# Asherchi/Stereo_Match_Traditional

Hardware: AMD Instinct MI355X
Metric: Mdisparities/s (HxWxD/s) + ms/pair, AD-Census 1920x1080 D=192 (higher is better)
Workload: dtype f32; 1 GPU; AD-Census 9x7 both views + WTA, 1920x1080 D=192 (adcensus_1080p_d192); parallelism=pairs sharded over 1 GPU(s), backend=none (single process), ranks_joined=1, ranks_joined_how=all_reduce(SUM) of 1 per rank over the job's communicator, world_size=1, launcher=none

## Files before the change

stereo_match_traditional_amd/csrc/adcensus.hip:

```cpp
#include "smt_common.h"
#include "adcensus_internal.h"
#include <math.h>
#include <stdlib.h>
#include <string.h>
#include <algorithm>
#include <new>
#include <type_traits>

namespace {

constexpr int TJ = 64;
constexpr int NT = 256;

struct Tables {
    uint64_t *cenA[2];
    uint64_t *cenX[2];
    uint64_t *mask;
    uint8_t *u8[2];
    float *lut;
    uint16_t *rank;
    int *flag;
    int WX;
    int edge_col;
    unsigned long long *stamp;
// ... 1257 lines not shown
        const vecf<C> x = *reinterpret_cast<const vecf<C> *>(c);
#pragma unroll
        for (int k = 0; k < C; k++) v[k] = x.v[k];
    } else {
#pragma unroll
        for (int k = 0; k < C; k++) v[k] = (dl + k < D) ? c[k] : INFINITY;
    }
    const int wd = wave_wta<C, FULL>(v, dl, D);
    if (lane == 0) disp[p] = (float)wd;
}

}

thread_local int g_smt_last_hip = 0;

struct smt_adcensus {
    int device;
    int H, W, D;
    float sigmaC, sigmaS;
    hipStream_t stream;
    float *vol[2];
    Tables T;
    Tables TS[2];
    hipStream_t prep_stream;
    hipEvent_t in_ready, prep_done[2], cost_done[2];
    long n_pairs;
    hipEvent_t *ev;
    bool timing;
    bool force_generic;
    long n_timed;
    long n_seen;
    int timing_stride;
    bool *ev_merged;
    bool plain_stores;
    float store_mode_ms[2];
    int place_tries;
    float place_ms;
    unsigned long long *skeys[2];
    bool conv_pending;
    int conv_map;
    float *conv_dR;
    bool vol_lent, vol_pending;
    int maps_resident[3];
};

SMT_API const char *smt_strerror(int s)
{
    switch (s) {
    case SMT_OK: return "ok";
    case SMT_ERR_ARG: return "invalid argument";
    case SMT_ERR_HIP: return "HIP runtime error";
    case SMT_ERR_ALLOC: return "device allocation failed";
    case SMT_ERR_DOMAIN: return "image values outside the integer 0..255 domain";
    case SMT_ERR_REF_UB: return "reference behaviour undefined for these inputs";
    case SMT_ERR_STATE: return "call order violated";
    default: return "unknown status";
// ... 180 lines not shown
            kv[a * 64 + c] = ((uint64_t)bits << 32) | (uint32_t)(a * 64 + c);
        }
    std::sort(kv, kv + RANK_N);
    int r = -1;
    uint32_t prev = 0;
    for (int n = 0; n < RANK_N; n++) {
        const uint32_t bits = (uint32_t)(kv[n] >> 32);
        if (n == 0 || bits != prev) r++;
        prev = bits;
        rank[(uint32_t)kv[n]] = (uint16_t)r;
    }
    delete[] kv;
    return true;
}

static void flush_conversion(smt_adcensus *h)
{
    if (!h->conv_pending) return;
    const long N = (long)h->H * h->W;
    hipLaunchKernelGGL(k_shared_convert, dim3((unsigned)shared_conv_items(h->H, h->W)), dim3(NT), 0, h->stream,
                       h->skeys[h->conv_map], h->conv_dR, N);
    h->conv_pending = false;
}

template <int C, bool FULL>
static void query_maps_resident(smt_adcensus *h, int cus)
{
    int n[3] = {0, 0, 0};
    if (hipOccupancyMaxActiveBlocksPerMultiprocessor(&n[0], k_cost_maps_shared<C, FULL>, NT, 0) != hipSuccess) n[0] = 0;
    if (hipOccupancyMaxActiveBlocksPerMultiprocessor(&n[1], k_cost_maps2p<C, FULL, MODE_MAPS_FLOAT>, NT, 0) != hipSuccess) n[1] = 0;
    if (hipOccupancyMaxActiveBlocksPerMultiprocessor(&n[2], k_cost_maps2p<C, FULL, MODE_MAPS_RANK>, NT, 0) != hipSuccess) n[2] = 0;
    for (int t = 0; t < 3; t++) h->maps_resident[t] = n[t] > 0 ? cus / 8 * n[t] : 0;
}
static void set_maps_resident(smt_adcensus *h)
{
    h->maps_resident[0] = h->maps_resident[1] = h->maps_resident[2] = 0;
    int cus = 0;
// ... 10 lines not shown
    default: break;
    }
    (void)hipGetLastError();
}

static int adcensus_create(int H, int W, int D, float sigmaC, float sigmaS, unsigned flags, smt_adcensus **out)
{
    if (!out || H <= 0 || W <= 0 || D <= 0 || D > SMT_MAX_DISPARITY || !(sigmaC > 0.0f) || !(sigmaS > 0.0f) ||
        (long long)H * W >= (1ll << 31))
        return SMT_ERR_ARG;
    smt_adcensus *h = new (std::nothrow) smt_adcensus();
    if (!h) return SMT_ERR_ALLOC;
    h->device = smt_current_device();
    h->H = H; h->W = W; h->D = D; h->sigmaC = sigmaC; h->sigmaS = sigmaS;
    h->stream = nullptr; h->timing = false; h->force_generic = false; h->ev = nullptr; h->n_timed = 0; h->n_seen = 0; h->timing_stride = 1; h->ev_merged = nullptr;
    h->n_pairs = 0;
    const size_t N = (size_t)H * W, V = N * D;
    const int WX = W + 4;
    int rc = place_volumes(h, !(flags & SMT_ADCENSUS_NO_PLACEMENT_SEARCH));
    auto alloc = [&](void **p, size_t bytes) { if (rc == SMT_OK) rc = smt_malloc(p, bytes); };
    alloc((void **)&h->TS[0].lut, 320 * 4);
    alloc((void **)&h->TS[0].rank, RANK_N * 2);
    alloc((void **)&h->TS[0].flag, 4);
    for (int t = 0; t < 2; t++) {
        h->TS[t].WX = WX;
        h->TS[t].stamp = nullptr;
        h->TS[t].lut = h->TS[0].lut;
        h->TS[t].rank = h->TS[0].rank;
        h->TS[t].flag = h->TS[0].flag;
        for (int v = 0; v < 2; v++) {
            alloc((void **)&h->TS[t].cenA[v], N * 8);
            alloc((void **)&h->TS[t].cenX[v], (size_t)H * WX * 8);
            alloc((void **)&h->TS[t].u8[v], N);
        }
        alloc((void **)&h->TS[t].mask, N * 8);
    }
    for (int t = 0; t < 2; t++) alloc((void **)&h->skeys[t], N * 8);
    h->T = h->TS[0];
    if (rc != SMT_OK) { smt_adcensus_destroy(h); return rc; }
    if (hipStreamCreateWithFlags(&h->prep_stream, hipStreamNonBlocking) != hipSuccess ||
        hipEventCreateWithFlags(&h->in_ready, hipEventDisableTiming) != hipSuccess) {
        smt_adcensus_destroy(h);
        return SMT_ERR_HIP;
    }
    for (int t = 0; t < 2; t++)
        if (hipEventCreateWithFlags(&h->prep_done[t], hipEventDisableTiming) != hipSuccess ||
            hipEventCreateWithFlags(&h->cost_done[t], hipEventDisableTiming) != hipSuccess) {
            smt_adcensus_destroy(h);
            return SMT_ERR_HIP;
        }
    float lut[320];
    build_lut(sigmaC, sigmaS, lut);
    uint16_t *rank = new (std::nothrow) uint16_t[RANK_N];
    if (!rank || !build_rank(lut, rank)) { delete[] rank; smt_adcensus_destroy(h); return SMT_ERR_ALLOC; }
    const bool rank_ok = hipMemcpy(h->TS[0].rank, rank, RANK_N * 2, hipMemcpyHostToDevice) == hipSuccess;
    delete[] rank;
    if (!rank_ok || hipMemcpy(h->TS[0].lut, lut, sizeof(lut), hipMemcpyHostToDevice) != hipSuccess ||
        hipMemset(h->vol[0], 0, V * 4) != hipSuccess || hipMemset(h->vol[1], 0, V * 4) != hipSuccess ||
        hipMemset(h->TS[0].flag, 0, 4) != hipSuccess || hipMemset(h->skeys[0], 0xFF, N * 8) != hipSuccess ||
        hipMemset(h->skeys[1], 0xFF, N * 8) != hipSuccess) {
        smt_adcensus_destroy(h);
        return SMT_ERR_HIP;
    }
    calibrate_store_mode(h, !(flags & SMT_ADCENSUS_NO_STORE_CALIBRATION));
    set_maps_resident(h);
    *out = h;
    return SMT_OK;
}

SMT_API int smt_adcensus_create(int H, int W, int D, float sigmaC, float sigmaS, smt_adcensus **out)
{
    return adcensus_create(H, W, D, sigmaC, sigmaS, 0u, out);
}

SMT_API int smt_adcensus_create_ex(int device, int H, int W, int D, float sigmaC, float sigmaS, unsigned flags, smt_adcensus **out)
{
    if (flags & ~(unsigned)(SMT_ADCENSUS_NO_PLACEMENT_SEARCH | SMT_ADCENSUS_NO_STORE_CALIBRATION)) return SMT_ERR_ARG;
    if (device < 0) return adcensus_create(H, W, D, sigmaC, sigmaS, flags, out);
// ... 3 lines not shown
    return adcensus_create(H, W, D, sigmaC, sigmaS, flags, out);
}

SMT_API int smt_adcensus_create_on(int device, int H, int W, int D, float sigmaC, float sigmaS, smt_adcensus **out)
{
    int n = 0;
    if (hipGetDeviceCount(&n) != hipSuccess || device < 0 || device >= n) return SMT_ERR_ARG;
    smt_dev_guard dev_guard(device);
    return smt_adcensus_create(H, W, D, sigmaC, sigmaS, out);
}

SMT_API int smt_adcensus_destroy(smt_adcensus *h)
{
    if (!h) return SMT_ERR_ARG;
    smt_dev_guard dev_guard(h->device);
    if (h->conv_pending) { flush_conversion(h); (void)hipStreamSynchronize(h->stream); }
    if (h->prep_stream) { (void)hipStreamSynchronize(h->prep_stream); (void)hipStreamDestroy(h->prep_stream); }
    if (h->in_ready) (void)hipEventDestroy(h->in_ready);
    for (int t = 0; t < 2; t++) {
        if (h->prep_done[t]) (void)hipEventDestroy(h->prep_done[t]);
        if (h->cost_done[t]) (void)hipEventDestroy(h->cost_done[t]);
    }
    (void)hipFree(h->vol[0]); (void)hipFree(h->vol[1]);
    for (int t = 0; t < 2; t++) {
        for (int v = 0; v < 2; v++) {
            (void)hipFree(h->TS[t].cenA[v]); (void)hipFree(h->TS[t].cenX[v]); (void)hipFree(h->TS[t].u8[v]);
        }
        (void)hipFree(h->TS[t].mask);
    }
    (void)hipFree(h->TS[0].lut); (void)hipFree(h->TS[0].rank); (void)hipFree(h->TS[0].flag);
    (void)hipFree(h->skeys[0]); (void)hipFree(h->skeys[1]);
    if (h->ev) {
        for (int k = 0; k < SMT_TIMING_SLOTS * 4; k++) (void)hipEventDestroy(h->ev[k]);
        delete[] h->ev_merged;
        delete[] h->ev;
    }
    delete h;
    return SMT_OK;
}

SMT_API int smt_adcensus_set_stream(smt_adcensus *h, void *s)
{
    if (!h) return SMT_ERR_ARG;
    smt_dev_guard dev_guard(h->device);
    h->stream = smt_stream(s);
    return SMT_OK;
}

SMT_API int smt_adcensus_set_quirks(smt_adcensus *h, unsigned quirks)
{
    if (!h || (quirks & ~SMT_QUIRK_FIX_ALL)) return SMT_ERR_ARG;
    const int col = (quirks & SMT_QUIRK_FIX_CENSUS_RIGHT_EDGE) ? h->W - 1 : 0;
    h->T.edge_col = h->TS[0].edge_col = h->TS[1].edge_col = col;
    return SMT_OK;
}

template <int C, bool FULL>
static void launch_cost(smt_adcensus *h, int view0, int nviews, float *d0, float *d1)
{
    const int D = h->D;
    dim3 grid((h->W + TJ - 1) / TJ, h->H, nviews);
    const int NX = TJ + D;
    size_t shm = (size_t)NX * 8 + TJ * 16 + 320 * 4 + NX + TJ;
    shm = (shm + 15) & ~(size_t)15;
    hipLaunchKernelGGL((k_cost<C, FULL>), grid, dim3(NT), shm, h->stream, h->H, h->W, D, h->T,
                       view0, h->vol[0], h->vol[1], d0, d1);
}

static int maps_chunks()
{
    const char *env = getenv("SMT_MAPS_CHUNKS");
    const int k = env ? atoi(env) : 0;
    return k >= 1 && k <= 64 ? k : 4;
}

constexpr int TAPER_N2_HALVES = 0, TAPER_N1_HALVES = 2;
static void maps_taper(int S, long per, int K, int &n2, int &n1)
{
    n2 = n1 = 0;
    const char *env = getenv("SMT_MAPS_TAPER");
// ... 32 lines not shown
    return !(env && env[0] == 'r') && dL && dR && maps_shared_shape(h->W, h->D) && maps_shared();
}

static int prep_items(int H, int W, int &ptx)
{
    ptx = (W + PTW - 1) / PTW;
    const int pty = (H + PTH - 1) / PTH, eb = (H + PNT / 16 - 1) / (PNT / 16);
    return ptx * (pty + (eb + ptx - 1) / ptx);
}

template <int C, bool FULL>
static void launch_fast(smt_adcensus *h, int views, float *dL, float *dR, const float *nL, const float *nR, bool maps)
{
    const int nbx = (h->W + FTJ - 1) / FTJ;
    auto blocks = [&](int nviews) { return dim3((unsigned)(((long)nbx * h->H * nviews + 7) / 8 * 8)); };
    if (views == SMT_VIEW_BOTH && maps) {
        const int K = maps_chunks();
        int nprep = 0, ptx = 1;
        if (nL) nprep = prep_items(h->H, h->W, ptx);
        const Tables &Tn = h->TS[(h->n_pairs + 1) & 1];
        const char *env = getenv("SMT_MAPS_KERNEL");
        int n2, n1;
        if (pair_takes_shared(h, views, dL, dR, maps)) {
            const int km = (int)(h->n_pairs & 1);
            if (h->conv_pending && h->conv_map == km) flush_conversion(h);
            const bool carried = h->conv_pending;
            maps_taper(h->maps_resident[0], ((long)nbx * h->H + 7) >> 3, K, n2, n1);
            const int ncs = maps_groups(nbx, h->H, 1, K, n2, n1), Dd = FULL ? 64 * C : h->D;
            const int cbody = maps_body_groups(nbx, h->H, 1, K, n2, n1);
            const int nconv = carried ? shared_conv_items(h->H, h->W) : 0, nedge = shared_edge_items(h->H, h->W, Dd);
            const unsigned gs = 8u * (unsigned)fused_grid(ncs, nprep + nconv + nedge, cbody).groups;
            hipLaunchKernelGGL((k_cost_maps_shared<C, FULL>), dim3(gs), dim3(NT), 0, h->stream, h->H, h->W, h->D, h->T, dL, dR,
                               h->skeys[km], nbx, K, shared_pub_hi(h->W), ncs, nprep, nL, nR, Tn, ptx, nconv, nedge,
                               carried ? h->skeys[h->conv_map] : nullptr, carried ? h->conv_dR : nullptr, n2, n1, cbody);
            if (SMT_SHARED_KNOCKOUT != 2) { h->conv_pending = true; h->conv_map = km; h->conv_dR = dR; }
            else h->conv_pending = false;
            if (shared_finish_apart()) flush_conversion(h);
            return;
        }
        const bool rank = env && env[0] == 'r';
        maps_taper(h->maps_resident[rank ? 2 : 1], ((long)nbx * h->H * 2 + 7) >> 3, K, n2, n1);
        const int ncost = maps_groups(nbx, h->H, 2, K, n2, n1), cbody = maps_body_groups(nbx, h->H, 2, K, n2, n1);
        const unsigned grid = nL ? 8u * (unsigned)fused_grid(ncost, nprep, cbody).groups : (unsigned)ncost;
        if (rank)
            hipLaunchKernelGGL((k_cost_maps2p<C, FULL, MODE_MAPS_RANK>), dim3(grid), dim3(NT), 0, h->stream, h->H, h->W,
                               h->D, h->T, dL, dR, nbx, K, ncost, nprep, nL, nR, Tn, ptx, n2, n1, cbody);
        else
            hipLaunchKernelGGL((k_cost_maps2p<C, FULL, MODE_MAPS_FLOAT>), dim3(grid), dim3(NT), 0, h->stream, h->H, h->W,
                               h->D, h->T, dL, dR, nbx, K, ncost, nprep, nL, nR, Tn, ptx, n2, n1, cbody);
        return;
    }
    if (views == SMT_VIEW_BOTH && nL) {
        const int ncost = (int)blocks(2).x;
        const int ptx = (h->W + PTW - 1) / PTW, pty = (h->H + PTH - 1) / PTH;
        const int eb = (h->H + PNT / 16 - 1) / (PNT / 16);
        const int nprep = ptx * (pty + (eb + ptx - 1) / ptx);
        const unsigned grid = 8u * (unsigned)fused_grid(ncost, nprep).groups;
        const Tables &Tn = h->TS[(h->n_pairs + 1) & 1];
        if (h->plain_stores)
            hipLaunchKernelGGL((k_cost_fast2p<C, FULL, false>), dim3(grid), dim3(NT), 0, h->stream, h->H, h->W, h->D, h->T,
                               h->vol[0], h->vol[1], dL, dR, nbx, ncost, nprep, nL, nR, Tn, ptx);
        else
            hipLaunchKernelGGL((k_cost_fast2p<C, FULL, true>), dim3(grid), dim3(NT), 0, h->stream, h->H, h->W, h->D, h->T,
                               h->vol[0], h->vol[1], dL, dR, nbx, ncost, nprep, nL, nR, Tn, ptx);
        return;
    }
    if (views == SMT_VIEW_BOTH) {
        if (h->plain_stores)
            hipLaunchKernelGGL((k_cost_fast2<C, FULL, false>), blocks(2), dim3(NT), 0, h->stream, h->H, h->W, h->D, h->T, h->vol[0],
                               h->vol[1], dL, dR, nbx);
        else
            hipLaunchKernelGGL((k_cost_fast2<C, FULL, true>), blocks(2), dim3(NT), 0, h->stream, h->H, h->W, h->D, h->T, h->vol[0],
                               h->vol[1], dL, dR, nbx);
        return;
    }
    if (views & SMT_VIEW_LEFT)
        hipLaunchKernelGGL((k_cost_fast<C, 0, FULL>), blocks(1), dim3(NT), 0, h->stream, h->H, h->W, h->D, h->T,
                           h->vol[0], dL, nbx);
    if (views & SMT_VIEW_RIGHT)
        hipLaunchKernelGGL((k_cost_fast<C, 1, FULL>), blocks(1), dim3(NT), 0, h->stream, h->H, h->W, h->D, h->T,
                           h->vol[1], dR, nbx);
}

static bool launch_fast_as(int C, bool full, smt_adcensus *h, int views, float *dL, float *dR, const float *nL,
                           const float *nR, bool maps)
{
    switch (C * 2 + (full ? 1 : 0)) {
    case 3: launch_fast<1, true>(h, views, dL, dR, nL, nR, maps); break;
    case 5: launch_fast<2, true>(h, views, dL, dR, nL, nR, maps); break;
    case 7: launch_fast<3, true>(h, views, dL, dR, nL, nR, maps); break;
    case 9: launch_fast<4, true>(h, views, dL, dR, nL, nR, maps); break;
    case 2: launch_fast<1, false>(h, views, dL, dR, nL, nR, maps); break;
    case 4: launch_fast<2, false>(h, views, dL, dR, nL, nR, maps); break;
    case 6: launch_fast<3, false>(h, views, dL, dR, nL, nR, maps); break;
    case 8: launch_fast<4, false>(h, views, dL, dR, nL, nR, maps); break;
    default: return false;
    }
    return true;
}

static bool fast_both_views(const smt_adcensus *h, int views)
{
    return views == SMT_VIEW_BOTH && !h->force_generic && (h->D + 63) / 64 <= 4;
}

static int adcensus_pair(smt_adcensus *h, const float *L, const float *R, int views, float *dL,
                         float *dR, bool overlap, bool prepped = false, const float *nL = nullptr,
                         const float *nR = nullptr, bool maps = false)
{
    const int H = h->H, W = h->W, D = h->D;
    const int set = (int)(h->n_pairs & 1);
    h->T = h->TS[set];
    h->vol_pending = false;
    if (!pair_takes_shared(h, views, dL, dR, maps)) flush_conversion(h);
    const bool timed = h->timing && (h->n_seen++ % h->timing_stride) == 0;
    const long slot = h->n_timed % SMT_TIMING_SLOTS;
    hipEvent_t *ev = timed ? h->ev + 4 * slot : nullptr;
    hipStream_t ps = overlap ? h->prep_stream : h->stream;
    if (overlap && h->n_pairs >= 2) SMT_HIP(hipStreamWaitEvent(ps, h->cost_done[set], 0));
    if (timed) (void)hipEventRecord(ev[0], ps);
    if (!prepped) {
        const int tx = (W + PTW - 1) / PTW, ty = (H + PTH - 1) / PTH;
        const int eb = (H + PNT / 16 - 1) / (PNT / 16);
        hipLaunchKernelGGL(k_prep, dim3(tx, ty + (eb + tx - 1) / tx), dim3(PNT), 0, ps, L, R, H, W, h->T);
    }
    if (timed) (void)hipEventRecord(ev[1], ps);
    if (overlap) {
        SMT_HIP(hipEventRecord(h->prep_done[set], ps));
        SMT_HIP(hipStreamWaitEvent(h->stream, h->prep_done[set], 0));
    }
    if (timed) { h->ev_merged[slot] = !overlap; if (overlap) (void)hipEventRecord(ev[2], h->stream); }
    const int view0 = (views & SMT_VIEW_LEFT) ? 0 : 1;
    const int nviews = (views == SMT_VIEW_BOTH) ? 2 : 1;
    const int C = (D + 63) / 64;
    const bool full = (D % 64) == 0;
    if (h->force_generic || C > 4) {
        switch (C) {
        case 1: launch_cost<1, false>(h, view0, nviews, dL, dR); break;
        case 2: launch_cost<2, false>(h, view0, nviews, dL, dR); break;
        case 3: launch_cost<3, false>(h, view0, nviews, dL, dR); break;
        case 4: launch_cost<4, false>(h, view0, nviews, dL, dR); break;
        case 5: launch_cost<5, false>(h, view0, nviews, dL, dR); break;
        case 6: launch_cost<6, false>(h, view0, nviews, dL, dR); break;
        case 7: launch_cost<7, false>(h, view0, nviews, dL, dR); break;
        default: launch_cost<8, false>(h, view0, nviews, dL, dR); break;
        }
    } else if (!launch_fast_as(C, full, h, views, dL, dR, nL, nR, maps)) return SMT_ERR_ARG;
    if (timed) { (void)hipEventRecord(ev[3], h->stream); h->n_timed++; }
    if (!prepped && !nL) SMT_HIP(hipEventRecord(h->cost_done[set], h->stream));
    h->n_pairs++;
    SMT_LAUNCH_CHECK();
    return SMT_OK;
}

SMT_API int smt_adcensus_compute(smt_adcensus *h, const float *L, const float *R, int views,
                                 float *dispL, float *dispR)
{
    if (!h || !L || !R || views < 1 || views > 3) return SMT_ERR_ARG;
    smt_dev_guard dev_guard(h->device);
    return adcensus_pair(h, L, R, views, dispL, dispR, false);
}

static int batch_schedule(const smt_adcensus *h, int views)
{
    const char *env = getenv("SMT_OVERLAP");
    int want = 2;
    if (env && env[0] >= '0' && env[0] <= '2' && env[1] == 0) want = env[0] - '0';
    if (want == 2 && !fast_both_views(h, views)) want = 1;
    return want;
}

int adcensus_batch_pairs(smt_adcensus *h, const float *L, const float *R, int n, int views, float *dispL,
                         float *dispR, int sched, bool prepped, const float *nL, const float *nR, bool maps_ok,
                         bool last_volumes)
{
    const size_t N = (size_t)h->H * h->W;
    maps_ok = maps_ok && fast_both_views(h, views);
    for (int b = 0; b < n; b++) {
        const bool last = b + 1 == n;
        const float *bl = sched == 2 ? (last ? nL : L + (b + 1) * N) : nullptr;
        const float *br = sched == 2 ? (last ? nR : R + (b + 1) * N) : nullptr;
        int rc = adcensus_pair(h, L + b * N, R + b * N, views, dispL ? dispL + b * N : nullptr,
                               dispR ? dispR + b * N : nullptr, sched == 1 && b > 0, b > 0 ? sched == 2 : prepped,
                               bl, br, maps_ok && (!last || !last_volumes));
        if (rc != SMT_OK) { flush_conversion(h); return rc; }
    }
    flush_conversion(h);
    SMT_LAUNCH_CHECK();
    return SMT_OK;
}

bool adcensus_fused_both_views(const smt_adcensus *h) { return fast_both_views(h, SMT_VIEW_BOTH); }

static int materialise_volumes(smt_adcensus *h)
{
    flush_conversion(h);
    if (!h->vol_pending) return SMT_OK;
    const long slot = h->n_timed % SMT_TIMING_SLOTS;
    hipEvent_t *ev = h->timing ? h->ev + 4 * slot : nullptr;
    if (ev) { (void)hipEventRecord(ev[0], h->stream); (void)hipEventRecord(ev[1], h->stream); h->ev_merged[slot] = true; }
    if (!launch_fast_as((h->D + 63) / 64, h->D % 64 == 0, h, SMT_VIEW_BOTH, nullptr, nullptr))
        return SMT_ERR_STATE;
    if (ev) { (void)hipEventRecord(ev[3], h->stream); h->n_timed++; }
    h->vol_pending = false;
    SMT_LAUNCH_CHECK();
    SMT_HIP(hipStreamSynchronize(h->stream));
    return SMT_OK;
}

SMT_API int smt_adcensus_compute_batch(smt_adcensus *h, const float *L, const float *R, int pairs,
                                       int views, float *dispL, float *dispR)
// ... 374 lines not shown
        }
        if (expect != per) rc = SMT_ERR_STATE;
    }
    for (long c = 0; c < nb && rc == SMT_OK; c++) if (seen[c] != 1) rc = SMT_ERR_STATE;
    for (long b = 0; b < 8 * ng && rc == SMT_OK && nb <= (1L << 20); b++) {
        long first;
        int i = -1, bx = -1;
        const int m = maps_span(per, K, n2, n1, b >> 3, first), got = shared_wg_chunks(1, (int)nb, K, b, i, bx, n2, n1);
        const long c = (b & 7) * per + first, want = c >= nb ? 0 : (nb - c < m ? nb - c : m);
        if (got != want || (got > 0 && (i != c || bx != 0))) rc = SMT_ERR_STATE;
    }
    delete[] seen;
    return rc;
}

SMT_API int smt_adcensus_selftest_cost_rank(float sigmaC, float sigmaS)
{
    if (!(sigmaC > 0.0f) || !(sigmaS > 0.0f)) return SMT_ERR_ARG;
    float lut[320];
    build_lut(sigmaC, sigmaS, lut);
    uint16_t *rank = new (std::nothrow) uint16_t[RANK_N];
    float *sum = new (std::nothrow) float[RANK_N];
    float *uniq = new (std::nothrow) float[RANK_N];
    int rc = (rank && sum && uniq && build_rank(lut, rank)) ? SMT_OK : SMT_ERR_ALLOC;
    int nu = 0;
    if (rc == SMT_OK) {
        for (int e = 0; e < RANK_N; e++) {
            sum[e] = lut[e >> 6] + lut[256 + (e & 63)];
            uint32_t bits;
            memcpy(&bits, &sum[e], 4);
// ... 73 lines not shown
    unsigned long long *stamp = nullptr;
    unsigned long long *hs = nullptr;
    float *ratio = nullptr;
    ~DiagResources()
    {
        for (auto &x : e) if (x) (void)hipEventDestroy(x);
        if (stamp) (void)hipFree(stamp);
        delete[] hs;
        delete[] ratio;
    }
};
}

static int smt_adcensus_diag_impl(smt_adcensus *h, int reps, float *sclk_mhz, float *cost_ms, float *store_only_ms, DiagResources &res)
{
    if (h->n_pairs == 0) return SMT_ERR_STATE;
    const int D = h->D, C = D / 64;
    if (D % 64 != 0 || C < 1 || C > 4) return SMT_ERR_ARG;
    const int nbx = (h->W + FTJ - 1) / FTJ;
    const unsigned nblk = (unsigned)(((long)nbx * h->H * 2 + 7) / 8 * 8);
    hipEvent_t (&e)[3] = res.e;
    for (auto &x : e) SMT_HIP(hipEventCreate(&x));
    if (smt_malloc((void **)&res.stamp, (size_t)nblk * 32) != SMT_OK) return SMT_ERR_ALLOC;
    unsigned long long *stamp = res.stamp;
    SMT_HIP(hipMemsetAsync(stamp, 0, (size_t)nblk * 32, h->stream));
    Tables T = h->T;
    T.stamp = stamp;
    SMT_HIP(hipEventRecord(e[0], h->stream));
    for (int r = 0; r < reps; r++) {
        switch (C) {
        case 1: hipLaunchKernelGGL((k_store_only2<1>), dim3(nblk), dim3(NT), 0, h->stream, h->H, h->W, h->vol[0], h->vol[1], nbx); break;
// ... 84 lines not shown
```

stereo_match_traditional_amd/csrc/adcensus_internal.h:

```cpp
#pragma once
#include "smt_common.h"

int adcensus_batch_pairs(smt_adcensus *h, const float *L, const float *R, int n, int views, float *dispL,
                         float *dispR, int sched, bool prepped, const float *nL, const float *nR, bool maps_ok,
                         bool last_volumes);
bool adcensus_fused_both_views(const smt_adcensus *h);
SMT_API int smt_adcensus_selftest_shared_keys(int H, int W, int D, int K, unsigned seed);
SMT_API int smt_adcensus_selftest_shared_aux_grid(int ncost, int nprep, int nedge, int nconv);
SMT_API int smt_adcensus_selftest_shared_aux(int H, int W, int D, int K, int first, int last);
SMT_API int smt_adcensus_selftest_spans(long nb, int K, int n2, int n1);
```

Baseline: 2.036 million Mdisp/s.

## Run batched stereo pairs as concurrent chains across multiple streams

Adds a chained batch schedule (sched==3) that splits the pairs of a batch into up to three independent chains. Each chain has its own census/mask table sets, shared-key buffers and conversion state, and runs on its own stream, with fork/join events keeping the order correct. The goal is to overlap kernels from different pairs so the GPU stays busy during tails and small prep/convert phases. In exchange it allocates more device buffers, and the kernels from concurrent chains compete for compute units. The maps taper is disabled when chains run side by side. A host-side selftest checks that the plan's dependencies are sound.

```diff
diff --git a/stereo_match_traditional_amd/csrc/adcensus.hip b/stereo_match_traditional_amd/csrc/adcensus.hip
--- a/stereo_match_traditional_amd/csrc/adcensus.hip
+++ b/stereo_match_traditional_amd/csrc/adcensus.hip
@@ -5,6 +5,7 @@
 #include <string.h>
 #include <algorithm>
 #include <new>
+#include <vector>
 #include <type_traits>
 
 namespace {
@@ -1295,6 +1296,17 @@
 
 thread_local int g_smt_last_hip = 0;
 
+constexpr int SMT_MAX_CHAINS = 3;
+constexpr int SMT_CHAINS_DEFAULT = 2;
+constexpr bool SMT_CHAINED_DEFAULT = true;
+struct ChainState {
+    long n_pairs;
+    bool conv_pending;
+    int conv_map;
+    float *conv_dR;
+};
+static inline int chain_slot(int c, long n) { return 2 * c + (int)(n & 1); }
+
 struct smt_adcensus {
     int device;
     int H, W, D;
@@ -1302,10 +1314,14 @@
     hipStream_t stream;
     float *vol[2];
     Tables T;
-    Tables TS[2];
+    Tables TS[2 * SMT_MAX_CHAINS];
     hipStream_t prep_stream;
+    hipStream_t chain2_stream;
     hipEvent_t in_ready, prep_done[2], cost_done[2];
-    long n_pairs;
+    hipEvent_t fork_ev, join_ev[SMT_MAX_CHAINS];
+    ChainState chain[SMT_MAX_CHAINS];
+    int cur, chain_on[SMT_MAX_CHAINS];
+    bool beside;
     hipEvent_t *ev;
     bool timing;
     bool force_generic;
@@ -1317,10 +1333,7 @@
     float store_mode_ms[2];
     int place_tries;
     float place_ms;
-    unsigned long long *skeys[2];
-    bool conv_pending;
-    int conv_map;
-    float *conv_dR;
+    unsigned long long *skeys[2 * SMT_MAX_CHAINS];
     bool vol_lent, vol_pending;
     int maps_resident[3];
 };
@@ -1531,13 +1544,20 @@
     return true;
 }
 
-static void flush_conversion(smt_adcensus *h)
-{
-    if (!h->conv_pending) return;
+static hipStream_t chain_stream(const smt_adcensus *h, int c)
+{
+    return h->chain_on[c] == 0 ? h->stream : h->chain_on[c] == 1 ? h->prep_stream : h->chain2_stream;
+}
+static hipStream_t run_stream(const smt_adcensus *h) { return chain_stream(h, h->cur); }
+
+static void flush_conversion(smt_adcensus *h, int c)
+{
+    ChainState &ch = h->chain[c];
+    if (!ch.conv_pending) return;
     const long N = (long)h->H * h->W;
-    hipLaunchKernelGGL(k_shared_convert, dim3((unsigned)shared_conv_items(h->H, h->W)), dim3(NT), 0, h->stream,
-                       h->skeys[h->conv_map], h->conv_dR, N);
-    h->conv_pending = false;
+    hipLaunchKernelGGL(k_shared_convert, dim3((unsigned)shared_conv_items(h->H, h->W)), dim3(NT), 0, chain_stream(h, c),
+                       h->skeys[ch.conv_map], ch.conv_dR, N);
+    ch.conv_pending = false;
 }
 
 template <int C, bool FULL>
@@ -1578,7 +1598,6 @@
     h->device = smt_current_device();
     h->H = H; h->W = W; h->D = D; h->sigmaC = sigmaC; h->sigmaS = sigmaS;
     h->stream = nullptr; h->timing = false; h->force_generic = false; h->ev = nullptr; h->n_timed = 0; h->n_seen = 0; h->timing_stride = 1; h->ev_merged = nullptr;
-    h->n_pairs = 0;
     const size_t N = (size_t)H * W, V = N * D;
     const int WX = W + 4;
     int rc = place_volumes(h, !(flags & SMT_ADCENSUS_NO_PLACEMENT_SEARCH));
@@ -1586,7 +1605,7 @@
     alloc((void **)&h->TS[0].lut, 320 * 4);
     alloc((void **)&h->TS[0].rank, RANK_N * 2);
     alloc((void **)&h->TS[0].flag, 4);
-    for (int t = 0; t < 2; t++) {
+    for (int t = 0; t < 2 * SMT_MAX_CHAINS; t++) {
         h->TS[t].WX = WX;
         h->TS[t].stamp = nullptr;
         h->TS[t].lut = h->TS[0].lut;
@@ -1599,14 +1618,21 @@
         }
         alloc((void **)&h->TS[t].mask, N * 8);
     }
-    for (int t = 0; t < 2; t++) alloc((void **)&h->skeys[t], N * 8);
+    for (int t = 0; t < 2 * SMT_MAX_CHAINS; t++) alloc((void **)&h->skeys[t], N * 8);
     h->T = h->TS[0];
     if (rc != SMT_OK) { smt_adcensus_destroy(h); return rc; }
     if (hipStreamCreateWithFlags(&h->prep_stream, hipStreamNonBlocking) != hipSuccess ||
-        hipEventCreateWithFlags(&h->in_ready, hipEventDisableTiming) != hipSuccess) {
+        hipStreamCreateWithFlags(&h->chain2_stream, hipStreamNonBlocking) != hipSuccess ||
+        hipEventCreateWithFlags(&h->in_ready, hipEventDisableTiming) != hipSuccess ||
+        hipEventCreateWithFlags(&h->fork_ev, hipEventDisableTiming) != hipSuccess) {
         smt_adcensus_destroy(h);
         return SMT_ERR_HIP;
     }
+    for (int c = 1; c < SMT_MAX_CHAINS; c++)
+        if (hipEventCreateWithFlags(&h->join_ev[c], hipEventDisableTiming) != hipSuccess) {
+            smt_adcensus_destroy(h);
+            return SMT_ERR_HIP;
+        }
     for (int t = 0; t < 2; t++)
         if (hipEventCreateWithFlags(&h->prep_done[t], hipEventDisableTiming) != hipSuccess ||
             hipEventCreateWithFlags(&h->cost_done[t], hipEventDisableTiming) != hipSuccess) {
@@ -1621,11 +1647,12 @@
     delete[] rank;
     if (!rank_ok || hipMemcpy(h->TS[0].lut, lut, sizeof(lut), hipMemcpyHostToDevice) != hipSuccess ||
         hipMemset(h->vol[0], 0, V * 4) != hipSuccess || hipMemset(h->vol[1], 0, V * 4) != hipSuccess ||
-        hipMemset(h->TS[0].flag, 0, 4) != hipSuccess || hipMemset(h->skeys[0], 0xFF, N * 8) != hipSuccess ||
-        hipMemset(h->skeys[1], 0xFF, N * 8) != hipSuccess) {
+        hipMemset(h->TS[0].flag, 0, 4) != hipSuccess) {
         smt_adcensus_destroy(h);
         return SMT_ERR_HIP;
     }
+    for (int t = 0; t < 2 * SMT_MAX_CHAINS; t++)
+        if (hipMemset(h->skeys[t], 0xFF, N * 8) != hipSuccess) { smt_adcensus_destroy(h); return SMT_ERR_HIP; }
     calibrate_store_mode(h, !(flags & SMT_ADCENSUS_NO_STORE_CALIBRATION));
     set_maps_resident(h);
     *out = h;
@@ -1659,22 +1686,27 @@
 {
     if (!h) return SMT_ERR_ARG;
     smt_dev_guard dev_guard(h->device);
-    if (h->conv_pending) { flush_conversion(h); (void)hipStreamSynchronize(h->stream); }
+    for (int c = 0; c < SMT_MAX_CHAINS; c++)
+        if (h->chain[c].conv_pending) { flush_conversion(h, c); (void)hipStreamSynchronize(h->stream); }
     if (h->prep_stream) { (void)hipStreamSynchronize(h->prep_stream); (void)hipStreamDestroy(h->prep_stream); }
+    if (h->chain2_stream) { (void)hipStreamSynchronize(h->chain2_stream); (void)hipStreamDestroy(h->chain2_stream); }
     if (h->in_ready) (void)hipEventDestroy(h->in_ready);
+    if (h->fork_ev) (void)hipEventDestroy(h->fork_ev);
+    for (int c = 1; c < SMT_MAX_CHAINS; c++)
+        if (h->join_ev[c]) (void)hipEventDestroy(h->join_ev[c]);
     for (int t = 0; t < 2; t++) {
         if (h->prep_done[t]) (void)hipEventDestroy(h->prep_done[t]);
         if (h->cost_done[t]) (void)hipEventDestroy(h->cost_done[t]);
     }
     (void)hipFree(h->vol[0]); (void)hipFree(h->vol[1]);
-    for (int t = 0; t < 2; t++) {
+    for (int t = 0; t < 2 * SMT_MAX_CHAINS; t++) {
         for (int v = 0; v < 2; v++) {
             (void)hipFree(h->TS[t].cenA[v]); (void)hipFree(h->TS[t].cenX[v]); (void)hipFree(h->TS[t].u8[v]);
         }
         (void)hipFree(h->TS[t].mask);
     }
     (void)hipFree(h->TS[0].lut); (void)hipFree(h->TS[0].rank); (void)hipFree(h->TS[0].flag);
-    (void)hipFree(h->skeys[0]); (void)hipFree(h->skeys[1]);
+    for (int t = 0; t < 2 * SMT_MAX_CHAINS; t++) (void)hipFree(h->skeys[t]);
     if (h->ev) {
         for (int k = 0; k < SMT_TIMING_SLOTS * 4; k++) (void)hipEventDestroy(h->ev[k]);
         delete[] h->ev_merged;
@@ -1696,7 +1728,8 @@
 {
     if (!h || (quirks & ~SMT_QUIRK_FIX_ALL)) return SMT_ERR_ARG;
     const int col = (quirks & SMT_QUIRK_FIX_CENSUS_RIGHT_EDGE) ? h->W - 1 : 0;
-    h->T.edge_col = h->TS[0].edge_col = h->TS[1].edge_col = col;
+    h->T.edge_col = col;
+    for (int t = 0; t < 2 * SMT_MAX_CHAINS; t++) h->TS[t].edge_col = col;
     return SMT_OK;
 }
 
@@ -1708,7 +1741,7 @@
     const int NX = TJ + D;
     size_t shm = (size_t)NX * 8 + TJ * 16 + 320 * 4 + NX + TJ;
     shm = (shm + 15) & ~(size_t)15;
-    hipLaunchKernelGGL((k_cost<C, FULL>), grid, dim3(NT), shm, h->stream, h->H, h->W, D, h->T,
+    hipLaunchKernelGGL((k_cost<C, FULL>), grid, dim3(NT), shm, run_stream(h), h->H, h->W, D, h->T,
                        view0, h->vol[0], h->vol[1], d0, d1);
 }
 
@@ -1771,39 +1804,41 @@
 {
     const int nbx = (h->W + FTJ - 1) / FTJ;
     auto blocks = [&](int nviews) { return dim3((unsigned)(((long)nbx * h->H * nviews + 7) / 8 * 8)); };
+    ChainState &ch = h->chain[h->cur];
+    const hipStream_t st = run_stream(h);
     if (views == SMT_VIEW_BOTH && maps) {
         const int K = maps_chunks();
         int nprep = 0, ptx = 1;
         if (nL) nprep = prep_items(h->H, h->W, ptx);
-        const Tables &Tn = h->TS[(h->n_pairs + 1) & 1];
+        const Tables &Tn = h->TS[chain_slot(h->cur, ch.n_pairs + 1)];
         const char *env = getenv("SMT_MAPS_KERNEL");
         int n2, n1;
         if (pair_takes_shared(h, views, dL, dR, maps)) {
-            const int km = (int)(h->n_pairs & 1);
-            if (h->conv_pending && h->conv_map == km) flush_conversion(h);
-            const bool carried = h->conv_pending;
-            maps_taper(h->maps_resident[0], ((long)nbx * h->H + 7) >> 3, K, n2, n1);
+            const int km = chain_slot(h->cur, ch.n_pairs);
+            if (ch.conv_pending && ch.conv_map == km) flush_conversion(h, h->cur);
+            const bool carried = ch.conv_pending;
+            maps_taper(h->beside ? 0 : h->maps_resident[0], ((long)nbx * h->H + 7) >> 3, K, n2, n1);
             const int ncs = maps_groups(nbx, h->H, 1, K, n2, n1), Dd = FULL ? 64 * C : h->D;
             const int cbody = maps_body_groups(nbx, h->H, 1, K, n2, n1);
             const int nconv = carried ? shared_conv_items(h->H, h->W) : 0, nedge = shared_edge_items(h->H, h->W, Dd);
             const unsigned gs = 8u * (unsigned)fused_grid(ncs, nprep + nconv + nedge, cbody).groups;
-            hipLaunchKernelGGL((k_cost_maps_shared<C, FULL>), dim3(gs), dim3(NT), 0, h->stream, h->H, h->W, h->D, h->T, dL, dR,
+            hipLaunchKernelGGL((k_cost_maps_shared<C, FULL>), dim3(gs), dim3(NT), 0, st, h->H, h->W, h->D, h->T, dL, dR,
                                h->skeys[km], nbx, K, shared_pub_hi(h->W), ncs, nprep, nL, nR, Tn, ptx, nconv, nedge,
-                               carried ? h->skeys[h->conv_map] : nullptr, carried ? h->conv_dR : nullptr, n2, n1, cbody);
-            if (SMT_SHARED_KNOCKOUT != 2) { h->conv_pending = true; h->conv_map = km; h->conv_dR = dR; }
-            else h->conv_pending = false;
-            if (shared_finish_apart()) flush_conversion(h);
+                               carried ? h->skeys[ch.conv_map] : nullptr, carried ? ch.conv_dR : nullptr, n2, n1, cbody);
+            if (SMT_SHARED_KNOCKOUT != 2) { ch.conv_pending = true; ch.conv_map = km; ch.conv_dR = dR; }
+            else ch.conv_pending = false;
+            if (shared_finish_apart()) flush_conversion(h, h->cur);
             return;
         }
         const bool rank = env && env[0] == 'r';
-        maps_taper(h->maps_resident[rank ? 2 : 1], ((long)nbx * h->H * 2 + 7) >> 3, K, n2, n1);
+        maps_taper(h->beside ? 0 : h->maps_resident[rank ? 2 : 1], ((long)nbx * h->H * 2 + 7) >> 3, K, n2, n1);
         const int ncost = maps_groups(nbx, h->H, 2, K, n2, n1), cbody = maps_body_groups(nbx, h->H, 2, K, n2, n1);
         const unsigned grid = nL ? 8u * (unsigned)fused_grid(ncost, nprep, cbody).groups : (unsigned)ncost;
         if (rank)
-            hipLaunchKernelGGL((k_cost_maps2p<C, FULL, MODE_MAPS_RANK>), dim3(grid), dim3(NT), 0, h->stream, h->H, h->W,
+            hipLaunchKernelGGL((k_cost_maps2p<C, FULL, MODE_MAPS_RANK>), dim3(grid), dim3(NT), 0, st, h->H, h->W,
                                h->D, h->T, dL, dR, nbx, K, ncost, nprep, nL, nR, Tn, ptx, n2, n1, cbody);
         else
-            hipLaunchKernelGGL((k_cost_maps2p<C, FULL, MODE_MAPS_FLOAT>), dim3(grid), dim3(NT), 0, h->stream, h->H, h->W,
+            hipLaunchKernelGGL((k_cost_maps2p<C, FULL, MODE_MAPS_FLOAT>), dim3(grid), dim3(NT), 0, st, h->H, h->W,
                                h->D, h->T, dL, dR, nbx, K, ncost, nprep, nL, nR, Tn, ptx, n2, n1, cbody);
         return;
     }
@@ -1813,29 +1848,29 @@
         const int eb = (h->H + PNT / 16 - 1) / (PNT / 16);
         const int nprep = ptx * (pty + (eb + ptx - 1) / ptx);
         const unsigned grid = 8u * (unsigned)fused_grid(ncost, nprep).groups;
-        const Tables &Tn = h->TS[(h->n_pairs + 1) & 1];
+        const Tables &Tn = h->TS[chain_slot(h->cur, ch.n_pairs + 1)];
         if (h->plain_stores)
-            hipLaunchKernelGGL((k_cost_fast2p<C, FULL, false>), dim3(grid), dim3(NT), 0, h->stream, h->H, h->W, h->D, h->T,
+            hipLaunchKernelGGL((k_cost_fast2p<C, FULL, false>), dim3(grid), dim3(NT), 0, st, h->H, h->W, h->D, h->T,
                                h->vol[0], h->vol[1], dL, dR, nbx, ncost, nprep, nL, nR, Tn, ptx);
         else
-            hipLaunchKernelGGL((k_cost_fast2p<C, FULL, true>), dim3(grid), dim3(NT), 0, h->stream, h->H, h->W, h->D, h->T,
+            hipLaunchKernelGGL((k_cost_fast2p<C, FULL, true>), dim3(grid), dim3(NT), 0, st, h->H, h->W, h->D, h->T,
                                h->vol[0], h->vol[1], dL, dR, nbx, ncost, nprep, nL, nR, Tn, ptx);
         return;
     }
     if (views == SMT_VIEW_BOTH) {
         if (h->plain_stores)
-            hipLaunchKernelGGL((k_cost_fast2<C, FULL, false>), blocks(2), dim3(NT), 0, h->stream, h->H, h->W, h->D, h->T, h->vol[0],
+            hipLaunchKernelGGL((k_cost_fast2<C, FULL, false>), blocks(2), dim3(NT), 0, st, h->H, h->W, h->D, h->T, h->vol[0],
                                h->vol[1], dL, dR, nbx);
         else
-            hipLaunchKernelGGL((k_cost_fast2<C, FULL, true>), blocks(2), dim3(NT), 0, h->stream, h->H, h->W, h->D, h->T, h->vol[0],
+            hipLaunchKernelGGL((k_cost_fast2<C, FULL, true>), blocks(2), dim3(NT), 0, st, h->H, h->W, h->D, h->T, h->vol[0],
                                h->vol[1], dL, dR, nbx);
         return;
     }
     if (views & SMT_VIEW_LEFT)
-        hipLaunchKernelGGL((k_cost_fast<C, 0, FULL>), blocks(1), dim3(NT), 0, h->stream, h->H, h->W, h->D, h->T,
+        hipLaunchKernelGGL((k_cost_fast<C, 0, FULL>), blocks(1), dim3(NT), 0, st, h->H, h->W, h->D, h->T,
                            h->vol[0], dL, nbx);
     if (views & SMT_VIEW_RIGHT)
-        hipLaunchKernelGGL((k_cost_fast<C, 1, FULL>), blocks(1), dim3(NT), 0, h->stream, h->H, h->W, h->D, h->T,
+        hipLaunchKernelGGL((k_cost_fast<C, 1, FULL>), blocks(1), dim3(NT), 0, st, h->H, h->W, h->D, h->T,
                            h->vol[1], dR, nbx);
 }
 
@@ -1861,32 +1896,37 @@
     return views == SMT_VIEW_BOTH && !h->force_generic && (h->D + 63) / 64 <= 4;
 }
 
+static void launch_prep(const smt_adcensus *h, hipStream_t st, const float *L, const float *R, const Tables &T)
+{
+    const int tx = (h->W + PTW - 1) / PTW, ty = (h->H + PTH - 1) / PTH;
+    const int eb = (h->H + PNT / 16 - 1) / (PNT / 16);
+    hipLaunchKernelGGL(k_prep, dim3(tx, ty + (eb + tx - 1) / tx), dim3(PNT), 0, st, L, R, h->H, h->W, T);
+}
+
 static int adcensus_pair(smt_adcensus *h, const float *L, const float *R, int views, float *dL,
                          float *dR, bool overlap, bool prepped = false, const float *nL = nullptr,
                          const float *nR = nullptr, bool maps = false)
 {
-    const int H = h->H, W = h->W, D = h->D;
-    const int set = (int)(h->n_pairs & 1);
+    const int D = h->D;
+    ChainState &ch = h->chain[h->cur];
+    const int set = chain_slot(h->cur, ch.n_pairs);
+    const hipStream_t st = run_stream(h);
     h->T = h->TS[set];
     h->vol_pending = false;
-    if (!pair_takes_shared(h, views, dL, dR, maps)) flush_conversion(h);
+    if (!pair_takes_shared(h, views, dL, dR, maps)) flush_conversion(h, h->cur);
     const bool timed = h->timing && (h->n_seen++ % h->timing_stride) == 0;
     const long slot = h->n_timed % SMT_TIMING_SLOTS;
     hipEvent_t *ev = timed ? h->ev + 4 * slot : nullptr;
-    hipStream_t ps = overlap ? h->prep_stream : h->stream;
-    if (overlap && h->n_pairs >= 2) SMT_HIP(hipStreamWaitEvent(ps, h->cost_done[set], 0));
+    hipStream_t ps = overlap ? h->prep_stream : st;
+    if (overlap && ch.n_pairs >= 2) SMT_HIP(hipStreamWaitEvent(ps, h->cost_done[set], 0));
     if (timed) (void)hipEventRecord(ev[0], ps);
-    if (!prepped) {
-        const int tx = (W + PTW - 1) / PTW, ty = (H + PTH - 1) / PTH;
-        const int eb = (H + PNT / 16 - 1) / (PNT / 16);
-        hipLaunchKernelGGL(k_prep, dim3(tx, ty + (eb + tx - 1) / tx), dim3(PNT), 0, ps, L, R, H, W, h->T);
-    }
+    if (!prepped) launch_prep(h, ps, L, R, h->T);
     if (timed) (void)hipEventRecord(ev[1], ps);
     if (overlap) {
         SMT_HIP(hipEventRecord(h->prep_done[set], ps));
-        SMT_HIP(hipStreamWaitEvent(h->stream, h->prep_done[set], 0));
-    }
-    if (timed) { h->ev_merged[slot] = !overlap; if (overlap) (void)hipEventRecord(ev[2], h->stream); }
+        SMT_HIP(hipStreamWaitEvent(st, h->prep_done[set], 0));
+    }
+    if (timed) { h->ev_merged[slot] = !overlap; if (overlap) (void)hipEventRecord(ev[2], st); }
     const int view0 = (views & SMT_VIEW_LEFT) ? 0 : 1;
     const int nviews = (views == SMT_VIEW_BOTH) ? 2 : 1;
     const int C = (D + 63) / 64;
@@ -1903,9 +1943,9 @@
         default: launch_cost<8, false>(h, view0, nviews, dL, dR); break;
         }
     } else if (!launch_fast_as(C, full, h, views, dL, dR, nL, nR, maps)) return SMT_ERR_ARG;
-    if (timed) { (void)hipEventRecord(ev[3], h->stream); h->n_timed++; }
-    if (!prepped && !nL) SMT_HIP(hipEventRecord(h->cost_done[set], h->stream));
-    h->n_pairs++;
+    if (timed) { (void)hipEventRecord(ev[3], st); h->n_timed++; }
+    if (!prepped && !nL && h->cur == 0) SMT_HIP(hipEventRecord(h->cost_done[set], st));
+    ch.n_pairs++;
     SMT_LAUNCH_CHECK();
     return SMT_OK;
 }
@@ -1921,10 +1961,192 @@
 static int batch_schedule(const smt_adcensus *h, int views)
 {
     const char *env = getenv("SMT_OVERLAP");
-    int want = 2;
-    if (env && env[0] >= '0' && env[0] <= '2' && env[1] == 0) want = env[0] - '0';
-    if (want == 2 && !fast_both_views(h, views)) want = 1;
+    int want = SMT_CHAINED_DEFAULT ? 3 : 2;
+    if (env && env[0] >= '0' && env[0] <= '3' && env[1] == 0) want = env[0] - '0';
+    if (want >= 2 && !fast_both_views(h, views)) want = 1;
     return want;
+}
+
+enum { CH_PREP, CH_PAIR, CH_CONVERT, CH_RECORD, CH_WAIT };
+constexpr int SMT_CHAIN_TAPER_DEFAULT = 0;
+enum { CHAIN_ORDER_BESIDE = 0, CHAIN_ORDER_PAIRS, CHAIN_ORDER_AB, CHAIN_ORDER_BA };
+enum { CHAIN_SHARED = 1, CHAIN_LAST_VOLUMES = 2, CHAIN_FORK_START = 4, CHAIN_FINISH_APART = 8, CHAIN_FLAGS = 15 };
+struct ChainOp {
+    int kind;
+    int stream;
+    int chain;
+    int pair;
+    int ts_read;
+    int ts_built;
+    int built_for;
+    int key_merged;
+    int key_conv;
+    int conv_pair;
+    int ev;
+};
+
+static int chain_plan(int n, int nc, const long *count0, int order, unsigned flags, std::vector<ChainOp> &ops)
+{
+    ops.clear();
+    if (n < 1 || nc < 1 || nc > SMT_MAX_CHAINS || !count0 || order < CHAIN_ORDER_BESIDE || order > CHAIN_ORDER_BA ||
+        (flags & ~(unsigned)CHAIN_FLAGS))
+        return SMT_ERR_ARG;
+    long cnt[SMT_MAX_CHAINS];
+    int pend_key[SMT_MAX_CHAINS], pend_pair[SMT_MAX_CHAINS];
+    for (int c = 0; c < SMT_MAX_CHAINS; c++) {
+        if (count0[c] < 0) return SMT_ERR_ARG;
+        cnt[c] = count0[c]; pend_key[c] = pend_pair[c] = -1;
+    }
+    if (nc > n) nc = n;
+    auto on = [&](int c) { return order == CHAIN_ORDER_PAIRS ? 0 : c; };
+    auto blank = [&](int kind, int c) { return ChainOp{kind, on(c), c, -1, -1, -1, -1, -1, -1, -1, -1}; };
+    auto event = [&](int kind, int stream, int ev) {
+        if (order == CHAIN_ORDER_PAIRS || nc < 2) return;
+        ChainOp o = blank(kind, stream); o.stream = stream; o.ev = ev; ops.push_back(o);
+    };
+    auto prep = [&](int c) {
+        ChainOp o = blank(CH_PREP, c); o.pair = o.built_for = c; o.ts_built = chain_slot(c, cnt[c]); ops.push_back(o);
+    };
+    auto convert = [&](int c) {
+        if (pend_key[c] < 0) return;
+        ChainOp o = blank(CH_CONVERT, c); o.key_conv = pend_key[c]; o.conv_pair = pend_pair[c]; ops.push_back(o);
+        pend_key[c] = pend_pair[c] = -1;
+    };
+    auto pair = [&](int b) {
+        const int c = b % nc;
+        const bool shared = (flags & CHAIN_SHARED) && !(b + 1 == n && (flags & CHAIN_LAST_VOLUMES));
+        if (!shared) convert(c);
+        ChainOp o = blank(CH_PAIR, c);
+        o.pair = b; o.ts_read = chain_slot(c, cnt[c]);
+        if (b + nc < n) { o.ts_built = chain_slot(c, cnt[c] + 1); o.built_for = b + nc; }
+        if (shared) {
+            o.key_merged = chain_slot(c, cnt[c]); o.key_conv = pend_key[c]; o.conv_pair = pend_pair[c];
+            pend_key[c] = o.key_merged; pend_pair[c] = b;
+        }
+        ops.push_back(o);
+        cnt[c]++;
+        if (flags & CHAIN_FINISH_APART) convert(c);
+    };
+    auto whole_chain = [&](int c) { prep(c); for (int b = c; b < n; b += nc) pair(b); convert(c); };
+    switch (order) {
+    case CHAIN_ORDER_BESIDE: case CHAIN_ORDER_PAIRS:
+        if (flags & CHAIN_FORK_START) event(CH_RECORD, 0, 0);
+        prep(0);
+        if (!(flags & CHAIN_FORK_START)) event(CH_RECORD, 0, 0);
+        for (int c = 1; c < nc; c++) { event(CH_WAIT, c, 0); prep(c); }
+        for (int b = 0; b < n; b++) pair(b);
+        for (int c = 0; c < nc; c++) convert(c);
+        for (int c = 1; c < nc; c++) event(CH_RECORD, c, c);
+        for (int c = 1; c < nc; c++) event(CH_WAIT, 0, c);
+        break;
+    case CHAIN_ORDER_AB:
+        whole_chain(0);
+        event(CH_RECORD, 0, 0);
+        for (int c = 1; c < nc; c++) { event(CH_WAIT, c, c - 1); whole_chain(c); event(CH_RECORD, c, c); }
+        for (int c = 1; c < nc; c++) event(CH_WAIT, 0, c);
+        break;
+    default:
+        event(CH_RECORD, 0, 0);
+        for (int c = 1; c < nc; c++) { event(CH_WAIT, c, 0); whole_chain(c); event(CH_RECORD, c, c); }
+        for (int c = 1; c < nc; c++) event(CH_WAIT, 0, c);
+        whole_chain(0);
+        break;
+    }
+    return SMT_OK;
+}
+
+static int chain_count()
+{
+    const char *env = getenv("SMT_CHAINS");
+    return env && env[0] >= '1' && env[0] <= '0' + SMT_MAX_CHAINS && env[1] == 0 ? env[0] - '0' : SMT_CHAINS_DEFAULT;
+}
+static int chain_order()
+{
+    const char *env = getenv("SMT_CHAIN_ORDER");
+    if (!env) return CHAIN_ORDER_BESIDE;
+    return strcmp(env, "pairs") == 0 ? CHAIN_ORDER_PAIRS : strcmp(env, "ab") == 0 ? CHAIN_ORDER_AB :
+           strcmp(env, "ba") == 0 ? CHAIN_ORDER_BA : CHAIN_ORDER_BESIDE;
+}
+
+enum { CHAIN_TAPER_NONE, CHAIN_TAPER_LAST, CHAIN_TAPER_ALL };
+static int chain_taper()
+{
+    const char *env = getenv("SMT_CHAIN_TAPER");
+    if (!env) return SMT_CHAIN_TAPER_DEFAULT;
+    return strcmp(env, "all") == 0 ? CHAIN_TAPER_ALL : strcmp(env, "last") == 0 ? CHAIN_TAPER_LAST :
+           strcmp(env, "none") == 0 ? CHAIN_TAPER_NONE : SMT_CHAIN_TAPER_DEFAULT;
+}
+
+static int adcensus_batch_chained(smt_adcensus *h, const float *L, const float *R, int n, int views, float *dispL,
+                                  float *dispR, bool last_volumes)
+{
+    const size_t N = (size_t)h->H * h->W;
+    const char *fenv = getenv("SMT_CHAIN_FORK");
+    unsigned flags = 0;
+    if (pair_takes_shared(h, views, dispL, dispR, true)) flags |= CHAIN_SHARED;
+    if (last_volumes) flags |= CHAIN_LAST_VOLUMES;
+    if (fenv && strcmp(fenv, "start") == 0) flags |= CHAIN_FORK_START;
+    if (shared_finish_apart()) flags |= CHAIN_FINISH_APART;
+    long count0[SMT_MAX_CHAINS];
+    for (int c = 0; c < SMT_MAX_CHAINS; c++) count0[c] = h->chain[c].n_pairs;
+    std::vector<ChainOp> ops;
+    const int nc = chain_count(), order = chain_order(), taper = chain_taper();
+    int rc = chain_plan(n, nc, count0, order, flags, ops);
+    if (rc != SMT_OK) return rc;
+    const bool concurrent = order == CHAIN_ORDER_BESIDE && std::min(nc, n) >= 2;
+    auto internal = [&](int s) { return s == 1 ? h->prep_stream : h->chain2_stream; };
+    auto stream = [&](int s) { return s == 0 ? h->stream : internal(s); };
+    bool open[SMT_MAX_CHAINS] = {false, false, false};
+    int last_set = 0;
+    auto issue = [&](const ChainOp &o) -> int {
+        if (o.stream > 0 && o.kind != CH_RECORD) open[o.stream] = true;
+        h->cur = o.chain;
+        h->chain_on[o.chain] = o.kind == CH_RECORD || o.kind == CH_WAIT ? h->chain_on[o.chain] : o.stream;
+        switch (o.kind) {
+        case CH_PREP:
+            launch_prep(h, stream(o.stream), L + o.pair * N, R + o.pair * N, h->TS[o.ts_built]);
+            return SMT_OK;
+        case CH_PAIR: {
+            const int b = o.pair;
+            if (chain_slot(o.chain, h->chain[o.chain].n_pairs) != o.ts_read) return SMT_ERR_STATE;
+            if (b + 1 == n) last_set = o.ts_read;
+            h->beside = concurrent && (taper == CHAIN_TAPER_NONE || (taper == CHAIN_TAPER_LAST && b + 1 < n));
+            return adcensus_pair(h, L + b * N, R + b * N, views, dispL ? dispL + b * N : nullptr,
+                                 dispR ? dispR + b * N : nullptr, false, true,
+                                 o.ts_built >= 0 ? L + o.built_for * N : nullptr,
+                                 o.ts_built >= 0 ? R + o.built_for * N : nullptr, !(b + 1 == n && last_volumes));
+        }
+        case CH_CONVERT:
+            flush_conversion(h, o.chain);
+            return SMT_OK;
+        case CH_RECORD:
+            SMT_HIP(hipEventRecord(o.ev ? h->join_ev[o.ev] : h->fork_ev, stream(o.stream)));
+            if (o.stream > 0) open[o.stream] = false;
+            return SMT_OK;
+        default:
+            SMT_HIP(hipStreamWaitEvent(stream(o.stream), o.ev ? h->join_ev[o.ev] : h->fork_ev, 0));
+            return SMT_OK;
+        }
+    };
+    for (size_t k = 0; k < ops.size() && rc == SMT_OK; k++) rc = issue(ops[k]);
+    if (rc != SMT_OK) {
+        for (int c = 0; c < SMT_MAX_CHAINS; c++) flush_conversion(h, c);
+        for (int s = 1; s < SMT_MAX_CHAINS; s++) {
+            bool used = open[s];
+            for (int c = 0; c < SMT_MAX_CHAINS; c++) used = used || h->chain_on[c] == s;
+            if (!used) continue;
+            (void)hipEventRecord(h->join_ev[s], internal(s));
+            (void)hipStreamWaitEvent(h->stream, h->join_ev[s], 0);
+        }
+    } else {
+        h->T = h->TS[last_set];
+    }
+    h->cur = 0;
+    h->beside = false;
+    for (int c = 0; c < SMT_MAX_CHAINS; c++) h->chain_on[c] = 0;
+    if (rc != SMT_OK) return rc;
+    SMT_LAUNCH_CHECK();
+    return SMT_OK;
 }
 
 int adcensus_batch_pairs(smt_adcensus *h, const float *L, const float *R, int n, int views, float *dispL,
@@ -1933,6 +2155,11 @@
 {
     const size_t N = (size_t)h->H * h->W;
     maps_ok = maps_ok && fast_both_views(h, views);
+    if (sched == 3) {
+        if (maps_ok && n >= 2 && !prepped && !nL && !nR)
+            return adcensus_batch_chained(h, L, R, n, views, dispL, dispR, last_volumes);
+        sched = 2;
+    }
     for (int b = 0; b < n; b++) {
         const bool last = b + 1 == n;
         const float *bl = sched == 2 ? (last ? nL : L + (b + 1) * N) : nullptr;
@@ -1940,9 +2167,9 @@
         int rc = adcensus_pair(h, L + b * N, R + b * N, views, dispL ? dispL + b * N : nullptr,
                                dispR ? dispR + b * N : nullptr, sched == 1 && b > 0, b > 0 ? sched == 2 : prepped,
                                bl, br, maps_ok && (!last || !last_volumes));
-        if (rc != SMT_OK) { flush_conversion(h); return rc; }
-    }
-    flush_conversion(h);
+        if (rc != SMT_OK) { flush_conversion(h, 0); return rc; }
+    }
+    flush_conversion(h, 0);
     SMT_LAUNCH_CHECK();
     return SMT_OK;
 }
@@ -1951,7 +2178,7 @@
 
 static int materialise_volumes(smt_adcensus *h)
 {
-    flush_conversion(h);
+    flush_conversion(h, 0);
     if (!h->vol_pending) return SMT_OK;
     const long slot = h->n_timed % SMT_TIMING_SLOTS;
     hipEvent_t *ev = h->timing ? h->ev + 4 * slot : nullptr;
@@ -2356,6 +2583,81 @@
     return rc;
 }
 
+SMT_API int smt_adcensus_selftest_chains(int pairs, int chains, long c0, long c1, long c2, int order, unsigned flags)
+{
+    if (pairs < 1 || pairs > 512) return SMT_ERR_ARG;
+    const long count0[SMT_MAX_CHAINS] = {c0, c1, c2};
+    std::vector<ChainOp> ops;
+    const int prc = chain_plan(pairs, chains, count0, order, flags, ops);
+    if (prc != SMT_OK) return prc;
+    const int nc = std::min(chains, pairs);
+    const int m = (int)ops.size(), M = m + 2;
+    auto stream_of = [&](int k) { return k == 0 || k == M - 1 ? 0 : ops[k - 1].stream; };
+    std::vector<std::vector<unsigned char>> before(M, std::vector<unsigned char>(M, 0));
+    int last_on[SMT_MAX_CHAINS] = {-1, -1, -1}, recorded[SMT_MAX_CHAINS] = {-1, -1, -1};
+    auto edge = [&](int from, int to) {
+        for (int j = 0; j < M; j++) before[to][j] |= before[from][j];
+        before[to][from] = 1;
+    };
+    for (int k = 0; k < M; k++) {
+        const int s = stream_of(k);
+        if (s < 0 || s >= SMT_MAX_CHAINS) return SMT_ERR_STATE;
+        if (last_on[s] >= 0) edge(last_on[s], k);
+        last_on[s] = k;
+        if (k == 0 || k == M - 1) continue;
+        const ChainOp &o = ops[k - 1];
+        if (o.kind == CH_RECORD) recorded[o.ev] = k;
+        if (o.kind == CH_WAIT) {
+            if (recorded[o.ev] < 0) return SMT_ERR_STATE;
+            edge(recorded[o.ev], k);
+        }
+    }
+    auto hb = [&](int a, int b) { return before[b][a] != 0; };
+    for (int k = 1; k < M - 1; k++)
+        if (!hb(0, k) || !hb(k, M - 1)) return SMT_ERR_STATE;
+    std::vector<int> launches(pairs, 0), converted(pairs, 0);
+    for (int k = 1; k < M - 1; k++) {
+        const ChainOp &o = ops[k - 1];
+        if (o.kind == CH_PAIR) {
+            if (o.pair < 0 || o.pair >= pairs || o.chain != o.pair % nc) return SMT_ERR_STATE;
+            if (o.stream != (order == CHAIN_ORDER_PAIRS ? 0 : o.chain)) return SMT_ERR_STATE;
+            launches[o.pair]++;
+            int builder = -1;
+            for (int j = 1; j < M - 1; j++)
+                if (ops[j - 1].ts_built == o.ts_read && ops[j - 1].built_for == o.pair && hb(j, k)) builder = builder < 0 ? j : -2;
+            if (builder < 0) return SMT_ERR_STATE;
+            for (int j = 1; j < M - 1; j++)
+                if (j != builder && ops[j - 1].ts_built == o.ts_read && !hb(j, builder) && !hb(k, j)) return SMT_ERR_STATE;
+            if (o.key_merged >= 0 && o.key_merged == o.key_conv) return SMT_ERR_STATE;
+        }
+        if (o.key_conv >= 0) {
+            if (o.conv_pair < 0 || o.conv_pair >= pairs) return SMT_ERR_STATE;
+            converted[o.conv_pair]++;
+        }
+    }
+    const bool any_shared = (flags & CHAIN_SHARED) != 0;
+    for (int b = 0; b < pairs; b++) {
+        const bool shared = any_shared && !(b + 1 == pairs && (flags & CHAIN_LAST_VOLUMES));
+        if (launches[b] != 1 || converted[b] != (shared ? 1 : 0)) return SMT_ERR_STATE;
+    }
+    for (int key = 0; key < 2 * SMT_MAX_CHAINS; key++) {
+        int prev = -1, merged_by = -1;
+        for (int k = 1; k < M - 1; k++) {
+            const ChainOp &o = ops[k - 1];
+            if (o.key_conv == key) {
+                if (merged_by < 0 || o.conv_pair != merged_by || !hb(prev, k)) return SMT_ERR_STATE;
+                prev = k; merged_by = -1;
+            }
+            if (o.key_merged == key) {
+                if (merged_by >= 0 || (prev >= 0 && !hb(prev, k))) return SMT_ERR_STATE;
+                prev = k; merged_by = o.pair;
+            }
+        }
+        if (merged_by >= 0) return SMT_ERR_STATE;
+    }
+    return SMT_OK;
+}
+
 SMT_API int smt_adcensus_selftest_cost_rank(float sigmaC, float sigmaS)
 {
     if (!(sigmaC > 0.0f) || !(sigmaS > 0.0f)) return SMT_ERR_ARG;
@@ -2459,7 +2761,7 @@
 
 static int smt_adcensus_diag_impl(smt_adcensus *h, int reps, float *sclk_mhz, float *cost_ms, float *store_only_ms, DiagResources &res)
 {
-    if (h->n_pairs == 0) return SMT_ERR_STATE;
+    if (h->chain[0].n_pairs == 0) return SMT_ERR_STATE;
     const int D = h->D, C = D / 64;
     if (D % 64 != 0 || C < 1 || C > 4) return SMT_ERR_ARG;
     const int nbx = (h->W + FTJ - 1) / FTJ;
diff --git a/stereo_match_traditional_amd/csrc/adcensus_internal.h b/stereo_match_traditional_amd/csrc/adcensus_internal.h
--- a/stereo_match_traditional_amd/csrc/adcensus_internal.h
+++ b/stereo_match_traditional_amd/csrc/adcensus_internal.h
@@ -9,3 +9,4 @@
 SMT_API int smt_adcensus_selftest_shared_aux_grid(int ncost, int nprep, int nedge, int nconv);
 SMT_API int smt_adcensus_selftest_shared_aux(int H, int W, int D, int K, int first, int last);
 SMT_API int smt_adcensus_selftest_spans(long nb, int K, int n2, int n1);
+SMT_API int smt_adcensus_selftest_chains(int pairs, int chains, long c0, long c1, long c2, int order, unsigned flags);
```

Result: faster. 2.096 million Mdisp/s, median of 6 (+3.0%).
